# SaurabhIndi/unet-segmentation

Measured on AMD Instinct MI355X. Metric: training images/sec (512×512×1, batch=8) at 1/2/4/8 MI355X; IoU vs ref, higher is better.
Workload: dtype fp32; 1 GPU; U-Net train step 512x512x1, batch 8/GPU, fp32 GEMMs (fwd+WCE+bwd+SGD); global_batch=8, image=512, parallelism=dp1

## Files before the change

### include/unet_hip.h

```cpp
#ifndef UNET_HIP_H
#define UNET_HIP_H

#include <stddef.h>
#include <stdint.h>

#ifdef __cplusplus
extern "C" {
#endif

typedef void* unet_stream_t;

const char* unet_version(void);
const char* unet_last_error(void);

typedef struct unet_plan unet_plan;

unet_plan* unet_plan_create(int n, int c_in, int h, int w, int n_classes);

enum { UNET_PREC_FP32 = 0, UNET_PREC_BF16 = 1, UNET_PREC_BF16X3 = 2 };
unet_plan* unet_plan_create_ex(int n, int c_in, int h, int w, int n_classes, int precision);
int unet_plan_precision(const unet_plan* p);
void unet_plan_destroy(unet_plan* p);
int unet_plan_out_hw(const unet_plan* p, int* out_h, int* out_w);
size_t unet_plan_workspace_bytes(const unet_plan* p);
// ... 65 lines not shown
int unet_weight_map(const uint16_t* labels, int n, int h, int w, double w0, double sigma, float* weights,
                    double* weights64, void* ws, unet_stream_t stream);

size_t unet_weight_map_border_ws_bytes(int n, int h, int w);
int unet_weight_map_border(const uint16_t* labels, int n, int h, int w, double w0, double sigma, float* weights,
                           double* weights64, int32_t* d1sq, int32_t* d2sq, void* ws, unet_stream_t stream);

size_t unet_instance_masks_ws_bytes(int n, int h, int w);
int unet_instance_masks(const uint8_t* mask, int n, int h, int w, int min_size, uint16_t* labels, void* ws,
                        unet_stream_t stream);
size_t unet_rand_index_ws_bytes(int h, int w);
int unet_rand_index(const uint16_t* gt, const uint16_t* pred, int h, int w, double* out, void* ws,
                    unet_stream_t stream);

typedef struct unet_tracker unet_tracker;
unet_tracker* unet_tracker_create(int h, int w, double iou_track, double iou_division, int max_children);
void unet_tracker_destroy(unet_tracker* t);
size_t unet_tracker_ws_bytes(int h, int w);
int unet_tracker_add_frame(unet_tracker* t, const uint16_t* labels, int frame, void* ws, unet_stream_t stream);
int unet_tracker_step_host(unet_tracker* t, int frame, int n_curr, const int32_t* host_labels,
                           const int64_t* host_areas, const int64_t* host_inter);
int unet_tracker_num_tracks(const unet_tracker* t);
int unet_tracker_tracks(const unet_tracker* t, int32_t* host_out, int cap);
int unet_linear_sum_assignment(long long nr, long long nc, const double* host_cost, int64_t* host_row_ind,
                               int64_t* host_col_ind);

int unet_set_tuning(const char* key, int value);
size_t unet_tuning_report(char* buf, size_t len);
int unet_tuning_reset(void);
long long unet_slab_fallbacks(int reset);
long long unet_nondeterministic_sites(int reset);
long long unet_fused_bnb_sites(int reset);
long long unet_wgrad_oihw_sites(int reset);
int unet_tuning_save(const char* path);
int unet_tuning_load(const char* path);

int unet_conv3x3_fwd(const float* x, int n, int h, int w, int ci, const float* wt_oihw,
                     const float* bias, int co, const float* x_scale, const float* x_shift,
                     float* y, void* ws, unet_stream_t stream);
int unet_conv3x3_dgrad(const float* dy, int n, int h, int w, int ci, const float* wt_oihw,
                       int co, float* dx, void* ws, unet_stream_t stream);
int unet_conv3x3_wgrad(const float* x, const float* dy, int n, int h, int w, int ci, int co,
                       float* dw_oihw, float* db, void* ws, unet_stream_t stream);
size_t unet_conv_ws_bytes(int n, int h, int w, int ci, int co);
int unet_convT2_fwd(const float* x, int n, int h, int w, int ci, const float* wt, const float* bias,
                    int co, float* y, void* ws, unet_stream_t stream);
int unet_convT2_bwd(const float* x, const float* dy, int n, int h, int w, int ci, const float* wt,
                    int co, float* dx, float* dw, float* db, void* ws, unet_stream_t stream);
int unet_maxpool2_fwd(const float* x, int n, int h, int w, int c, float* y, uint8_t* arg,
                      unet_stream_t stream);
int unet_maxpool2_bwd(const float* dy, const uint8_t* arg, int n, int h, int w, int c, float* dx,
                      unet_stream_t stream);
int unet_bn_train_fwd(const float* x, int n, int h, int w, int c, const float* gamma,
                      const float* beta, float* running_mean, float* running_var, float* y,
                      float* save_mean, float* save_invstd, void* ws, unet_stream_t stream);
int unet_bn_train_bwd(const float* x, const float* dy, int n, int h, int w, int c,
                      const float* gamma, const float* save_mean, const float* save_invstd,
                      float* dx, float* dgamma, float* dbeta, void* ws, unet_stream_t stream);
size_t unet_bn_ws_bytes(int c);

size_t unet_bn_relu_ws_bytes(int n, int h, int w, int c);
int unet_bn_relu_fwd(const float* x, int n, int h, int w, int c, const float* gamma, const float* beta,
                     float* running_mean, float* running_var, int64_t* nbt, float momentum, float eps,
                     int training, int relu, float* y, float* save_mean, float* save_invstd, void* ws,
                     unet_stream_t stream);
int unet_bn_relu_bwd(const float* x, const float* y, const float* dy, int n, int h, int w, int c,
// ... 20 lines not shown
```

### unet-segmentation_amd/csrc/igemm.hip

```cpp
#include <algorithm>
#include <cstdio>
#include <cstdlib>

#include "gemm_common.h"
#include "ring_common.h"

namespace unet {
constexpr int igemm_minw(int BM, int BN, int WM, int WN, int BK) {
  const int lds = 2 * (BM + BN) * (BK + 4) * 4 + WM * 3 * BN * 4;
  int blocks = 163840 / lds;
  if (blocks > 8) blocks = 8;
  int w = blocks * WM * WN * 64 / 256;
  if (WM * WN >= 8 && w > 2) w = 2;
  return w < 1 ? 1 : (w > 8 ? 8 : w);
}

template <int BM, int BN, int WM, int WN, int BK, int ABL = 0, int PF = 1>
__global__ __launch_bounds__(WM * WN * 64, igemm_minw(BM, BN, WM, WN, BK)) void k_igemm(const IgemmArgs args) {
  constexpr int NT = WM * WN * 64;
  constexpr int LDK = BK + 4;
  constexpr int TM = BM / (WM * 32), TN = BN / (WN * 32);
  constexpr int C4 = BK / 4;
  constexpr int RPP = NT / C4;
  constexpr int AV = BM / RPP, BV = BN / RPP;
// ... 944 lines not shown
  return g_num_cus;
}

int ablation_env(const char* name) {
  const char* v = getenv(name);
  if (!v || !*v) return 0;
#ifdef UNET_ABLATIONS
  return atoi(v);
#else
  fprintf(stderr, "unet_hip: %s=%s ignored (timing ablations need a build with -DUNET_ABLATIONS: make ABLATIONS=1)\n",
          name, v);
  return 0;
#endif
}

static int env_int(const char* name, int dflt) {
  const char* v = getenv(name);
  return v ? atoi(v) : dflt;
}
int g_tune_igemm = env_int("UNET_IGEMM_VARIANT", -1);
int g_tune_wgrad = env_int("UNET_WGRAD_VARIANT", -1);
std::atomic<long long> g_slab_fallbacks{0};
int g_wino_max = env_int("UNET_WINO_MAX", 4);
int g_wino_dgrad_max = env_int("UNET_WINO_DGRAD_MAX", 4);
int g_wino_wgrad_max = env_int("UNET_WINO_WGRAD_MAX", 6);
int g_wino4_fwd_min_cg = env_int("UNET_WINO4_FWD_MIN_CG", 128);
int g_wino4_fwd_small_cg = env_int("UNET_WINO4_FWD_SMALL_CG", 0);
template <int BM, int BN, int WM, int WN, int BK>
static hipError_t go_igemm(const IgemmArgs& a, hipStream_t s) {
  if (a.N % BN != 0 || a.K % BK != 0 || a.a.Cg % BK != 0 || a.a.c_split % BK != 0) return hipErrorInvalidValue;
  if (a.batch > 1) {
    if (a.ksplit > 1 || a.batch_rows < 1) return hipErrorInvalidValue;
    dim3 grid((a.batch_rows + BM - 1) / BM, a.N / BN, a.batch);
    hipLaunchKernelGGL((k_igemm<BM, BN, WM, WN, BK>), grid, dim3(WM * WN * 64), 0, s, a);
    return hipGetLastError();
  }
  dim3 grid((a.M + BM - 1) / BM, a.N / BN, a.ksplit > 1 ? a.ksplit : 1);
  hipLaunchKernelGGL((k_igemm<BM, BN, WM, WN, BK>), grid, dim3(WM * WN * 64), 0, s, a);
  return hipGetLastError();
}

template <int BM, int BN, int WM, int WN>
static hipError_t go_igemm_g(const IgemmArgs& a, hipStream_t s) {
  if (a.N % BN != 0 || a.K % 16 != 0 || a.a.Cg % 16 != 0 || a.a.c_split % 16 != 0) return hipErrorInvalidValue;
  static bool attr = false;
  const size_t full = igemm_g_smem<BM, BN>(1024);
  if (!attr) {
    hipError_t e = hipFuncSetAttribute(reinterpret_cast<const void*>(&k_igemm_g<BM, BN, WM, WN>),
                                       hipFuncAttributeMaxDynamicSharedMemorySize, (int)full);
    if (e != hipSuccess) return e;
    attr = true;
  }
  const bool tf = a.a.s[0].scale != nullptr || (a.a.c_split < a.a.Cg && a.a.s[1].scale != nullptr);
  if (tf && a.a.Cg > 1024) return hipErrorInvalidValue;
  const size_t smem = igemm_g_smem<BM, BN>(tf ? a.a.Cg : 0);
  dim3 grid((a.M + BM - 1) / BM, a.N / BN, a.ksplit > 1 ? a.ksplit : 1);
  hipLaunchKernelGGL((k_igemm_g<BM, BN, WM, WN>), grid, dim3(WM * WN * 64), smem, s, a);
  return hipGetLastError();
}

template <int TH, int TW, int BN, int WM, int WN, int MINW>
static hipError_t go_halo32(const IgemmArgs& a, hipStream_t s) {
  if (a.b == nullptr || a.N % BN != 0 || a.a.Cg % 16 != 0 || a.a.c_split % 16 != 0 || a.a.taps_h != 3 ||
      a.a.taps_w != 3 || a.a.stride != 1 || a.K != 9 * a.a.Cg)
    return hipErrorInvalidValue;
  constexpr size_t smem = conv3_f32_smem<TH, TW, BN>();
// ... 351 lines not shown
```

### unet-segmentation_amd/csrc/ops.hip

```cpp
#include <algorithm>
#include <cerrno>
#include <string>

#include "../../include/unet_hip.h"
#include "unet_internal.h"

using namespace unet;

namespace unet {
extern int g_tune_igemm, g_tune_wgrad, g_autotune, g_force_split, g_force_tile, g_concurrent, g_wino_max,
    g_wino_dgrad_max, g_wino_wgrad_max, g_bf16_norm, g_bn_fold, g_wino4_fwd_min_cg, g_wino4_fwd_small_cg,
    g_maxpool_vec8, g_wgrad_fwd_u;
hipError_t launch_fill(float* p, size_t n, float v, hipStream_t s);
hipError_t launch_pair_sum(const double* st, int g, int c, float* out, hipStream_t s);
}

namespace {
thread_local std::string g_op_err;
inline size_t al256(size_t b) { return (b + 255) / 256 * 256; }
int g_op_prec = UNET_PREC_FP32;
int g_op_a16 = 0;

hipError_t op_b_to_bf16(IgemmArgs& a, size_t n, void* scratch, hipStream_t s) {
  if (g_op_prec == UNET_PREC_FP32) return hipSuccess;
// ... 4 lines not shown
  a.bl = bl;
  a.b = nullptr;
  return e;
}
}

namespace {
__global__ void k_relu_mask(const float* __restrict__ dy, const float* __restrict__ y, long long n4,
                            float* __restrict__ dz) {
  for (long long i = blockIdx.x * (long long)blockDim.x + threadIdx.x; i < n4; i += (long long)gridDim.x * blockDim.x) {
    const float4 g = reinterpret_cast<const float4*>(dy)[i], v = reinterpret_cast<const float4*>(y)[i];
    reinterpret_cast<float4*>(dz)[i] =
        make_float4(v.x > 0.f ? g.x : 0.f, v.y > 0.f ? g.y : 0.f, v.z > 0.f ? g.z : 0.f, v.w > 0.f ? g.w : 0.f);
  }
}

__global__ void k_bn_eval_stats(int C, const float* rm, const float* rv, float eps, float* mean, float* invstd) {
  const int c = blockIdx.x * blockDim.x + threadIdx.x;
  if (c >= C) return;
  mean[c] = rm[c];
  invstd[c] = (float)(1.0 / sqrt((double)rv[c] + (double)eps));
}
}

#define OPCK(x)                                                           \
  do {                                                                    \
    hipError_t e_ = (x);                                                  \
    if (e_ != hipSuccess) return e_ == hipErrorInvalidValue ? -EINVAL : -EIO; \
  } while (0)

extern "C" {

static size_t op_wino_bytes(int ci, int co) { return al256(sizeof(float) * 36 * (size_t)ci * co); }
static void op_set_wino(IgemmArgs& a, void* ws, size_t ws_bytes, int ci, int co) {
  a.wino_ws = reinterpret_cast<float*>(reinterpret_cast<char*>(ws) + ws_bytes - op_wino_bytes(ci, co));
  a.wino_ws_bytes = op_wino_bytes(ci, co);
}

static size_t op_wgrad_wino_bytes(int n, int h, int w, int ci, int co) {
  return al256(wino_ws_bytes_grid(n, h, w, ci, co));
}
static size_t op_wgrad_slab_bytes(int n, int h, int w, int ci, int co) {
  const long long t4 = (long long)n * ((h + 3) / 4) * ((w + 3) / 4);
  return al256(sizeof(float) * 64 * (size_t)std::min<long long>(64, (t4 + 255) / 256) * ci * co);
}
static size_t op_wgrad_extra_bytes(int n, int h, int w, int ci, int co) {
  const size_t b = op_wgrad_wino_bytes(n, h, w, ci, co) + op_wgrad_slab_bytes(n, h, w, ci, co);
  return b <= ((size_t)256 << 20) ? b : 0;
}

size_t unet_conv_ws_bytes(int n, int h, int w, int ci, int co) {
  const size_t wb = al256(sizeof(float) * 9 * (size_t)ci * co);
  const size_t pad = al256(sizeof(float) * (size_t)n * (h + 2) * (w + 2) * co);
  const size_t misc = al256(sizeof(float) * 4 * co) + al256(sizeof(double) * kStatGroups * 2 * co);
  const size_t x16 = al256(sizeof(uint16_t) * (size_t)n * h * w * ci);
  return 2 * wb + pad + misc + x16 + op_wgrad_extra_bytes(n, h, w, ci, co) + op_wino_bytes(ci, co);
}

int unet_conv3x3_fwd(const float* x, int n, int h, int w, int ci, const float* wt, const float* bias, int co,
                     const float* xs, const float* xb, float* y, void* ws, unet_stream_t st) {
  if (ci % 16 || co % 64 || h < 3 || w < 3) return -EINVAL;
  hipStream_t s = reinterpret_cast<hipStream_t>(st);
  float* wf = reinterpret_cast<float*>(ws);
  OPCK(launch_pack_conv(wt, co, ci, 3, 3, wf, nullptr, s));
  IgemmArgs a;
  Src x0;
  x0.ptr = x;
  x0.H = h;
  x0.W = w;
  x0.C = ci;
  x0.scale = xs;
  x0.shift = xb;
  if (g_op_prec == UNET_PREC_BF16 && g_op_a16) {
    const size_t wb = al256(sizeof(float) * 9 * (size_t)ci * co);
    const size_t off = 2 * wb + al256(sizeof(float) * (size_t)n * (h + 2) * (w + 2) * co) +
                       al256(sizeof(float) * 4 * co) + al256(sizeof(double) * kStatGroups * 2 * co);
    uint16_t* x16 = reinterpret_cast<uint16_t*>(reinterpret_cast<char*>(ws) + off);
    OPCK(launch_f2bf(x, x16, (size_t)n * h * w * ci, s));
    x0.ptr = reinterpret_cast<const float*>(x16);
    x0.h16 = 1;
  }
  a.a.s[0] = a.a.s[1] = x0;
  a.a.Cg = a.a.c_split = ci;
  a.a.taps_h = a.a.taps_w = 3;
  a.a.Hg = h - 2;
  a.a.Wg = w - 2;
  a.a.nimg = n;
  a.b = wf;
  a.M = n * (h - 2) * (w - 2);
  a.N = co;
  a.K = 9 * ci;
  a.e.bias = bias;
  a.e.d[0] = Dst{y, h - 2, w - 2, co, 0, 0};
  op_set_wino(a, ws, unet_conv_ws_bytes(n, h, w, ci, co), ci, co);
  OPCK(op_b_to_bf16(a, 9 * (size_t)ci * co, reinterpret_cast<char*>(ws) + al256(sizeof(float) * 9 * (size_t)ci * co),
                    s));
  OPCK(launch_igemm(a, s));
  return 0;
}

int unet_conv3x3_dgrad(const float* dy, int n, int h, int w, int ci, const float* wt, int co, float* dx, void* ws,
                       unet_stream_t st) {
  if (ci % 64 || co % 16 || h < 3 || w < 3) return -EINVAL;
  hipStream_t s = reinterpret_cast<hipStream_t>(st);
  char* p = reinterpret_cast<char*>(ws);
  const size_t wb = al256(sizeof(float) * 9 * (size_t)ci * co);
  float* wf = reinterpret_cast<float*>(p);
  float* wd = reinterpret_cast<float*>(p + wb);
  float* dyp = reinterpret_cast<float*>(p + 2 * wb);
  float* coef = reinterpret_cast<float*>(p + 2 * wb + al256(sizeof(float) * (size_t)n * (h + 2) * (w + 2) * co));
  OPCK(launch_pack_conv(wt, co, ci, 3, 3, wf, wd, s));
  OPCK(launch_fill(coef, co, 1.f, s));
  OPCK(launch_fill(coef + co, 3 * (size_t)co, 0.f, s));
  const int dy16 = g_op_prec == UNET_PREC_BF16 && g_op_a16;
  OPCK(launch_bnb_apply(dy, dy, coef, n, h - 2, w - 2, co, dyp, 2, s, dy16, 0));
  IgemmArgs a;
  Src d;
  d.ptr = dyp;
  d.h16 = dy16;
  d.H = h + 2;
  d.W = w + 2;
  d.C = co;
  a.a.s[0] = a.a.s[1] = d;
  a.a.Cg = a.a.c_split = co;
  a.a.taps_h = a.a.taps_w = 3;
  a.a.Hg = h;
  a.a.Wg = w;
  a.a.nimg = n;
  a.b = wd;
  a.M = n * h * w;
  a.N = ci;
  a.K = 9 * co;
  a.e.d[0] = Dst{dx, h, w, ci, 0, 0};
  op_set_wino(a, ws, unet_conv_ws_bytes(n, h, w, ci, co), ci, co);
  OPCK(op_b_to_bf16(a, 9 * (size_t)ci * co, wf, s));
  OPCK(launch_igemm(a, s));
  return 0;
}

int unet_conv3x3_wgrad(const float* x, const float* dy, int n, int h, int w, int ci, int co, float* dw, float* db,
                       void* ws, unet_stream_t st) {
  if (ci % 64 || co % 64 || h < 3 || w < 3) return -EINVAL;
  hipStream_t s = reinterpret_cast<hipStream_t>(st);
  char* p = reinterpret_cast<char*>(ws);
  const size_t wb = al256(sizeof(float) * 9 * (size_t)ci * co);
  float* dwp = reinterpret_cast<float*>(p);
  double* st2 = reinterpret_cast<double*>(p + 2 * wb + al256(sizeof(float) * (size_t)n * (h + 2) * (w + 2) * co) +
                                          al256(sizeof(float) * 4 * co));
  OPCK(hipMemsetAsync(dwp, 0, sizeof(float) * 9 * (size_t)ci * co, s));
  WgradArgs a;
  Src d;
  d.ptr = dy;
  d.H = h - 2;
  d.W = w - 2;
  d.C = co;
  a.ga.s[0] = a.ga.s[1] = d;
  a.ga.Cg = a.ga.c_split = co;
  a.ga.Hg = h - 2;
  a.ga.Wg = w - 2;
  a.ga.nimg = n;
  Src xs;
  xs.ptr = x;
  xs.H = h;
  xs.W = w;
  xs.C = ci;
  a.gb.s[0] = a.gb.s[1] = xs;
  a.gb.Cg = a.gb.c_split = ci;
// ... 320 lines not shown
                      unet_stream_t st) {
  OPCK(launch_sgd(p, g, buf, n, lr, mom, gscale, first, reinterpret_cast<hipStream_t>(st)));
  return 0;
}

int unet_iou_counts(const uint8_t* a, const uint8_t* b, size_t n, unsigned long long* out, unet_stream_t st) {
  OPCK(launch_iou(a, b, n, out, reinterpret_cast<hipStream_t>(st)));
  return 0;
}

int unet_set_tuning(const char* key, int value) {
  if (!key) return -EINVAL;
  const std::string k(key);
  if (k == "igemm_variant") g_tune_igemm = value;
  else if (k == "wgrad_variant") g_tune_wgrad = value;
  else if (k == "autotune") g_autotune = value;
  else if (k == "force_split") g_force_split = value;
  else if (k == "force_tile") g_force_tile = value;
  else if (k == "concurrent") g_concurrent = value;
  else if (k == "wino_max") g_wino_max = value;
  else if (k == "bf16_norm") g_bf16_norm = value;
  else if (k == "bn_fold") g_bn_fold = value != 0;
  else if (k == "wino_dgrad_max") g_wino_dgrad_max = value;
  else if (k == "wino_wgrad_max") g_wino_wgrad_max = value;
  else if (k == "wino4_fwd_min_cg") g_wino4_fwd_min_cg = value;
  else if (k == "wino4_fwd_small_cg") g_wino4_fwd_small_cg = value;
  else if (k == "op_a16") g_op_a16 = value != 0;
  else if (k == "maxpool_vec8") g_maxpool_vec8 = value;
  else if (k == "bnb_fuse") g_bnb_fuse = value;
  else if (k == "wgrad_early_u") g_wgrad_early_u = value;
  else if (k == "wgrad_fwd_u") g_wgrad_fwd_u = value;
  else if (k == "wgrad_plane") g_wgrad_plane = value;
  else if (k == "wgrad_oihw") g_wgrad_oihw = value;
  else if (k == "deterministic") g_deterministic = value != 0;
  else if (k == "op_precision") {
    if (value != UNET_PREC_FP32 && value != UNET_PREC_BF16 && value != UNET_PREC_BF16X3) return -EINVAL;
    g_op_prec = value;
  } else return -EINVAL;
  return 0;
}

int unet_tile_gather(const float* image, int c, int h, int w, int tile_in, int tile_out, int top, int left, int nx,
                     int first, int stride, int ntiles, float* tiles, unet_stream_t st) {
  if (!image || !tiles) return -EINVAL;
  OPCK(launch_tile_gather(image, c, h, w, tile_in, tile_out, top, left, nx, first, stride, ntiles, tiles,
                          reinterpret_cast<hipStream_t>(st)));
  return 0;
}

int unet_tile_scatter(const float* tile_logits, int k, int tile_out, int nx, int first, int stride, int ntiles, int h,
                      int w, float* logits, uint8_t* mask, unet_stream_t st) {
  if (!tile_logits) return -EINVAL;
  OPCK(launch_tile_scatter(tile_logits, k, tile_out, nx, first, stride, ntiles, h, w, logits, mask,
                           reinterpret_cast<hipStream_t>(st)));
  return 0;
}

size_t unet_instance_masks_ws_bytes(int n, int h, int w) {
  return n > 0 && h > 0 && w > 0 ? instance_masks_ws_bytes(n, h, w) : 0;
}

int unet_instance_masks(const uint8_t* mask, int n, int h, int w, int min_size, uint16_t* labels, void* ws,
                        unet_stream_t st) {
  if (!mask || !labels || !ws) return -EINVAL;
  OPCK(launch_instance_masks(mask, n, h, w, min_size, labels, ws, reinterpret_cast<hipStream_t>(st)));
  return 0;
// ... 66 lines not shown
```

### unet-segmentation_amd/csrc/plan.hip

```cpp
#include <cerrno>
#include <cstdio>
#include <cstdlib>
#include <cstring>
#include <algorithm>
#include <array>
#include <map>
#include <mutex>
#include <string>
#include <vector>

#include "../../include/unet_hip.h"
#include "unet_internal.h"

using namespace unet;

namespace unet {
extern int g_wino_max, g_wino_dgrad_max, g_wino_wgrad_max, g_wino4_fwd_min_cg, g_wino4_fwd_small_cg;
int g_autotune = getenv("UNET_AUTOTUNE") ? atoi(getenv("UNET_AUTOTUNE")) : 1;
int g_concurrent = getenv("UNET_CONCURRENT") ? atoi(getenv("UNET_CONCURRENT")) : 1;
int g_bf16_norm = getenv("UNET_BF16_NORM") ? atoi(getenv("UNET_BF16_NORM")) : 0;
int g_bn_fold = getenv("UNET_BN_FOLD") ? atoi(getenv("UNET_BN_FOLD")) : 1;
int g_force_split = 0;
int g_force_tile = 0;
int g_deterministic = getenv("UNET_DETERMINISTIC") ? atoi(getenv("UNET_DETERMINISTIC")) : 0;
// ... 1344 lines not shown
    return -EINVAL;
  }
  if (!p->side || !p->side_pending) return 0;
  CK(hipEventRecord(p->ev_join, p->side));
  CK(hipStreamWaitEvent(reinterpret_cast<hipStream_t>(stream), p->ev_join, 0));
  p->side_pending = false;
  return 0;
}

size_t unet_tuning_report(char* buf, size_t len) {
  std::string r;
  {
    std::lock_guard<std::mutex> lk(g_tune_mu);
    for (const auto& kv : g_tune_log) r += kv.second + "\n";
  }
  if (buf && len > 0) {
    const size_t k = std::min(len - 1, r.size());
    memcpy(buf, r.data(), k);
    buf[k] = 0;
  }
  return r.size() + 1;
}

long long unet_nondeterministic_sites(int reset) {
  return reset ? g_nondet_sites.exchange(0) : g_nondet_sites.load();
}

long long unet_fused_bnb_sites(int reset) {
  return reset ? unet::g_fused_bnb_sites.exchange(0) : unet::g_fused_bnb_sites.load();
}
long long unet_wgrad_oihw_sites(int reset) {
  return reset ? unet::g_wgrad_oihw_sites.exchange(0) : unet::g_wgrad_oihw_sites.load();
}
long long unet_slab_fallbacks(int reset) {
  return reset ? g_slab_fallbacks.exchange(0) : g_slab_fallbacks.load();
}

int unet_tuning_reset(void) {
  std::lock_guard<std::mutex> lk(g_tune_mu);
  g_tuned.clear();
  g_tune_log.clear();
  return 0;
}

int unet_tuning_save(const char* path) {
  if (!path) return -EINVAL;
  std::lock_guard<std::mutex> lk(g_tune_mu);
  FILE* f = fopen(path, "w");
  if (!f) return -errno;
  for (const auto& kv : g_tuned) fprintf(f, "%s\t%d\t%d\n", kv.first.c_str(), kv.second.tile, kv.second.split);
  fclose(f);
  return (int)g_tuned.size();
}

int unet_tuning_load(const char* path) {
  if (!path) return -EINVAL;
  std::lock_guard<std::mutex> lk(g_tune_mu);
  return tune_db_read(path, true);
}

int unet_plan_set_timing(unet_plan* p, int enable) {
  if (!p) return -EINVAL;
  p->timing = enable != 0;
  return 0;
}

// ... 65 lines not shown
```

### unet-segmentation_amd/csrc/unet_internal.h

```cpp
#pragma once
#include <hip/hip_runtime.h>
#include <cstddef>
#include <cstdint>
#include <atomic>
#include <string>
#include <vector>

namespace unet {

constexpr int kMaxInChannels = 4096;
constexpr int kMaxClassCount = 4096;

struct Src {
  const float* ptr = nullptr;
  int H = 0, W = 0, C = 0;
  int oy = 0, ox = 0;
  const float* scale = nullptr;
  const float* shift = nullptr;
  int h16 = 0;
};

struct Gather {
  Src s[2];
  int c_split = 0;
// ... 24 lines not shown
  const float* bn_shift = nullptr;
  const float* bn_mean = nullptr;
  const float* bn_invstd = nullptr;
  double* bstats = nullptr;
  double* colsum1 = nullptr;
};

constexpr int kStatGroups = 64;

struct IgemmArgs {
  Gather a;
  const float* b = nullptr;
  const uint16_t* bh = nullptr;
  const uint16_t* bl = nullptr;
  int M, N, K;
  Epilogue e;
  int ksplit = 1;
  float* slab = nullptr;
  float* wino_ws = nullptr;
  size_t wino_ws_bytes = 0;
  int batch = 1;
  int batch_rows = 0;
  long long batch_b = 0;
  struct { int tile = -1, split = 1; } wino_choice;
  int fwd = 0;
};

extern std::atomic<long long> g_slab_fallbacks;
extern int g_deterministic;
extern int g_bnb_fuse;
extern int g_wgrad_early_u;
extern int g_wgrad_plane;
extern int g_wgrad_oihw;
extern std::atomic<long long> g_nondet_sites;

struct WgradArgs {
  Gather ga;
  Gather gb;
  int Mo, No;
  int P;
  int pix_per_split;
  float* out;
  float* out_oihw = nullptr;
  float* slab = nullptr;
  size_t slab_bytes = 0;
  int accumulate = 0;
  int bf16 = 0;
  int split = 0;
  int batch = 1;
  long long batch_a = 0, batch_b = 0, batch_out = 0;
  float* wino_ws = nullptr;
  size_t wino_ws_bytes = 0;
  const float* vd_pre = nullptr;
  int u_ready = 0;
  int abl = 0;
};

struct GemmChoice {
  int tile = -1;
  int split = 1;
};

enum class IgemmFamily {
  Reg,
  Halo,
  Conv3Dma,
// ... 96 lines not shown
size_t bnb_wino6_vd_bytes(int n, int h, int w, int c);
hipError_t launch_bnb_wino6_dy(const float* dz, const float* y, const float* coef, int n, int h, int w, int c,
                               float* dypad, float* vd, hipStream_t s);
bool conv3_ring_fits(const IgemmArgs& a, const IgemmTile& t);
bool gemm_ring_fits(const IgemmArgs& a, const IgemmTile& t);
size_t conv3_flat_sk_slab_bytes(const IgemmArgs& a);
int num_cus();

int ablation_env(const char* name);
hipError_t launch_igemm(const IgemmArgs& a, hipStream_t s);
hipError_t launch_igemm_v(const IgemmArgs& a, hipStream_t s, GemmChoice c);
int igemm_heuristic_tile(const IgemmArgs& a);
bool igemm_tile_fits(const IgemmArgs& a, int tile);
long long igemm_tile_count(const IgemmArgs& a, int tile);
int igemm_tile_slots(int tile);
size_t igemm_slab_bytes(const IgemmArgs& a, int ksplit);
std::string igemm_key(const IgemmArgs& a);
std::string wgrad_key(const WgradArgs& a);
std::vector<GemmChoice> igemm_candidates(const IgemmArgs& a, size_t slab_bytes);
std::vector<GemmChoice> wgrad_candidates(const WgradArgs& a);
bool wgrad_choice_deterministic(const GemmChoice& g);
hipError_t launch_wgrad(const WgradArgs& a, hipStream_t s);
hipError_t launch_wgrad_v(const WgradArgs& a, hipStream_t s, GemmChoice c);
bool wgrad_tile_fits(const WgradArgs& a, int tile);
bool reg_tile_fits(const IgemmArgs& a, const IgemmTile& t);
bool halo_tile_fits(const IgemmArgs& a, const IgemmTile& t);
bool wgrad3_fits(const WgradArgs& a);
hipError_t launch_slab_reduce(const float* slab, int splits, int batch, size_t plane, long long batch_out, float* out,
                              hipStream_t s);
int wgrad_splits(const WgradArgs& a, const WgradTile& t, int per_cu, int& pps);
bool wgrad_slab_fits(const WgradArgs& a, int splits);
bool wgrad_plane_applies(const WgradArgs& a, int bm, int bn);
hipError_t launch_wgrad_plane(const WgradArgs& a, hipStream_t s, dim3 grid, int bm, int bn);
hipError_t launch_f2bf(const float* in, uint16_t* out, size_t n, hipStream_t s, uint16_t* lo = nullptr);

hipError_t launch_tile_gather(const float* img, int c, int h, int w, int ti, int to, int top, int left, int nx,
                              int first, int stride, int ntiles, float* tiles, hipStream_t s);
hipError_t launch_tile_scatter(const float* lt, int k, int to, int nx, int first, int stride, int ntiles, int h,
                               int w, float* full, uint8_t* mask, hipStream_t s);

size_t instance_masks_ws_bytes(int n, int h, int w);
hipError_t launch_instance_masks(const uint8_t* mask, int n, int h, int w, int min_size, uint16_t* out, void* ws,
                                 hipStream_t s);
size_t rand_index_ws_bytes(int h, int w);
hipError_t launch_rand_index(const uint16_t* g, const uint16_t* p, int h, int w, double* out, void* ws,
                             hipStream_t s);

void set_last_error(const std::string& s);

size_t weight_map_ws_bytes(int n);
hipError_t launch_weight_map(const uint16_t* lab, int n, int h, int w, double w0, double sigma, float* out,
                             double* out64, void* ws, hipStream_t s);
size_t weight_map_border_ws_bytes(int n, int h, int w);
hipError_t launch_weight_map_border(const uint16_t* lab, int n, int h, int w, double w0, double sigma, float* out,
                                    double* out64, int32_t* d1sq, int32_t* d2sq, void* ws, hipStream_t s);

size_t elastic_ws_bytes(int n, int h, int w);
hipError_t launch_elastic(const uint8_t* img, const uint16_t* lab, int n, int h, int w, const double* noise,
                          double alpha, double sigma, float* x_out, uint8_t* t_out, uint8_t* img_out, uint16_t* ids_out,
                          void* ws, hipStream_t s);

hipError_t launch_conv_first_fwd(const float* x_nchw, int n, int ci, int h, int w,
                                 const float* wt_oihw, const float* bias, int co, float* y,
                                 double* stats, hipStream_t s, int out_h16 = 0, int relu = 0);
hipError_t launch_fold_bn(const float* w, long long K, int rows, const float* scale, const float* shift,
                          const float* bias, float* wout, float* bias_out, hipStream_t s);
// ... 78 lines not shown
```

### unet-segmentation_amd/csrc/winograd.hip

```cpp
#include <algorithm>
#include <cstdlib>

#include "gemm_common.h"
#include "ring_common.h"

namespace unet {

__global__ void k_wino_w(const float* __restrict__ b, int N, int Cg, float* __restrict__ v) {
  const long long i = blockIdx.x * (long long)blockDim.x + threadIdx.x;
  if (i >= (long long)N * Cg) return;
  const int n = (int)(i / Cg), c = (int)(i - (long long)n * Cg);
  float g[3][3];
#pragma unroll
  for (int t = 0; t < 9; ++t) g[t / 3][t % 3] = b[((size_t)n * 9 + t) * Cg + c];
  float tg[4][3];
#pragma unroll
  for (int k = 0; k < 3; ++k) {
    tg[0][k] = g[0][k];
    tg[1][k] = 0.5f * (g[0][k] + g[1][k] + g[2][k]);
    tg[2][k] = 0.5f * (g[0][k] - g[1][k] + g[2][k]);
    tg[3][k] = g[2][k];
  }
  const size_t plane = (size_t)N * Cg, o = (size_t)n * Cg + c;
#pragma unroll
// ... 606 lines not shown
    }
  }
}

static size_t wino_bytes(int P, long long T, int Cg, int N) {
  auto al = [](size_t b) { return (b + 255) / 256 * 256; };
  return al((size_t)P * T * Cg * 4) + al((size_t)P * T * N * 4) + al((size_t)P * N * Cg * 4);
}
size_t wino_ws_bytes(long long T, int Cg, int N) { return wino_bytes(16, T, Cg, N); }
size_t wino_ws_bytes_grid(int nimg, int H, int W, int Cg, int N) {
  const long long t2 = (long long)nimg * ((H + 1) / 2) * ((W + 1) / 2);
  const long long t4 = (long long)nimg * ((H + 3) / 4) * ((W + 3) / 4);
  const long long t6 = (long long)nimg * ((H + 5) / 6) * ((W + 5) / 6);
  const size_t a = wino_bytes(16, t2, Cg, N), b = wino_bytes(36, t4, Cg, N), c = wino_bytes(64, t6, Cg, N);
  return std::max(a, std::max(b, c));
}

bool wino_applies(const IgemmArgs& a, int mt) {
  const Gather& g = a.a;
  if (a.b == nullptr || a.bh != nullptr || g.taps_h != 3 || g.taps_w != 3 || g.stride != 1 || a.K != 9 * g.Cg ||
      g.Cg % 4 || g.c_split % 4 || a.N % 64 || g.s[0].h16 || g.s[1].h16 || a.e.shuffle_co)
    return false;
  for (int k = 0; k < 2; ++k) {
    const Dst& d = a.e.d[k];
    if (k == 1 && a.e.n_split >= a.N) break;
    if (d.h16 || d.oy || d.ox || d.H != g.Hg || d.W != g.Wg || d.C % 4) return false;
  }
  if (a.e.yref_h16 || a.e.n_split % 4) return false;
  const long long T = (long long)g.nimg * ((g.Hg + mt - 1) / mt) * ((g.Wg + mt - 1) / mt);
  if ((long long)(mt + 2) * (mt + 2) * T * std::max(g.Cg, a.N) * 4 >= (1ll << 32)) return false;
  return a.wino_ws != nullptr && wino_bytes((mt + 2) * (mt + 2), T, g.Cg, a.N) <= a.wino_ws_bytes;
}

hipError_t launch_wino(const IgemmArgs& a, hipStream_t s, int mt) {
  if (!wino_applies(a, mt)) return hipErrorInvalidValue;
  const Gather& g = a.a;
  const int P = (mt + 2) * (mt + 2);
  const int Th = (g.Hg + mt - 1) / mt, Tw = (g.Wg + mt - 1) / mt;
  const long long T = (long long)g.nimg * Th * Tw;
  char* w = reinterpret_cast<char*>(a.wino_ws);
  auto al = [](size_t b) { return (b + 255) / 256 * 256; };
  float* U = reinterpret_cast<float*>(w);
  float* Mm = reinterpret_cast<float*>(w + al((size_t)P * T * g.Cg * 4));
  float* V = reinterpret_cast<float*>(w + al((size_t)P * T * g.Cg * 4) + al((size_t)P * T * a.N * 4));
  const long long nw = (long long)a.N * g.Cg;
  if (mt == 2) {
    hipLaunchKernelGGL(k_wino_w, dim3((unsigned)((nw + 255) / 256)), dim3(256), 0, s, a.b, a.N, g.Cg, V);
    const long long ni = T * (g.Cg / 4);
    hipLaunchKernelGGL(k_wino_in, dim3((unsigned)((ni + 255) / 256)), dim3(256), 0, s, g, Th, Tw, T, U);
  } else if (mt == 4) {
    hipLaunchKernelGGL(k_wino4_w, dim3((unsigned)((nw + 255) / 256)), dim3(256), 0, s, a.b, a.N, g.Cg, V);
    launch_wino4_in(g, Th, Tw, T, U, s);
  } else {
    hipLaunchKernelGGL(k_wino6_w, dim3((unsigned)((nw + 255) / 256)), dim3(256), 0, s, a.b, a.N, g.Cg, V);
    launch_wino6_in(g, Th, Tw, T, U, s);
  }
  hipError_t e = hipGetLastError();
  if (e != hipSuccess) return e;
  {
    IgemmArgs q;
    Src u;
    u.ptr = U;
    u.H = 1;
    u.W = (int)(P * T);
    u.C = g.Cg;
    q.a.s[0] = q.a.s[1] = u;
    q.a.Cg = q.a.c_split = g.Cg;
    q.a.taps_h = q.a.taps_w = 1;
    q.a.Hg = 1;
    q.a.Wg = (int)(P * T);
    q.a.nimg = 1;
    q.b = V;
    q.M = (int)(P * T);
    q.N = a.N;
    q.K = g.Cg;
    q.e.d[0] = Dst{Mm, 1, (int)(P * T), a.N, 0, 0};
    q.batch = P;
    q.batch_rows = (int)T;
    q.batch_b = (long long)a.N * g.Cg;
    int tile = a.wino_choice.tile;
    if (tile <= 0 || !igemm_tile_fits(q, tile)) {
      const long long t256 = ((T + 255) / 256) * (a.N / 128) * P;
      tile = (a.N % 128 == 0 && t256 >= 2 * num_cus()) ? 4 : (a.N % 128 == 0 ? 1 : 8);
    }
    if ((e = launch_igemm_v(q, s, GemmChoice{tile, 1})) != hipSuccess) return e;
  }
  if (mt == 2) {
    const int C4 = a.N / 4, cgs = C4 < 64 ? C4 : 64, lanes = 256 / cgs;
    long long gx = (T + lanes * 4 - 1) / (lanes * 4);
    if (gx > 65535) gx = 65535;
    dim3 grid((unsigned)gx, (unsigned)((C4 + cgs - 1) / cgs));
    hipLaunchKernelGGL(k_wino_out, grid, dim3(256), 0, s, Mm, T, Th, Tw, a.N, g, a.e);
  } else {
    long long gx = (T + 15) / 16;
    if (gx > 65535) gx = 65535;
    dim3 grid((unsigned)gx, (unsigned)((a.N + 63) / 64));
    if (mt == 4) hipLaunchKernelGGL(k_wino4_out, grid, dim3(256), 0, s, Mm, T, Th, Tw, a.N, g, a.e);
    else hipLaunchKernelGGL(k_wino6_out, grid, dim3(256), 0, s, Mm, T, Th, Tw, a.N, g, a.e);
  }
  return hipGetLastError();
}

template <int CK>
__global__ void k_wino4f_w(const float* __restrict__ b, int N, int Cg, float* __restrict__ v) {
  const long long i = blockIdx.x * (long long)blockDim.x + threadIdx.x;
  if (i >= (long long)N * Cg) return;
  const int n = (int)(i / Cg), c = (int)(i - (long long)n * Cg);
  float tg[6][3];
#pragma unroll
  for (int k = 0; k < 3; ++k) {
    float col[3] = {b[((size_t)n * 9 + 0 + k) * Cg + c], b[((size_t)n * 9 + 3 + k) * Cg + c],
                    b[((size_t)n * 9 + 6 + k) * Cg + c]};
    float r[6];
// ... 1546 lines not shown
```

### unet-segmentation_amd/unet_amd/_lib.py

```python
from __future__ import annotations

import ctypes
import os

_HERE = os.path.dirname(os.path.abspath(__file__))
LIB_PATH = os.environ.get("UNET_HIP_LIB", os.path.join(_HERE, "libunet_hip.so"))

_vp = ctypes.c_void_p
_i = ctypes.c_int
_f = ctypes.c_float
_sz = ctypes.c_size_t

SIGNATURES = {
    "unet_version": (ctypes.c_char_p, []),
    "unet_last_error": (ctypes.c_char_p, []),
    "unet_plan_create": (_vp, [_i, _i, _i, _i, _i]),
    "unet_plan_create_ex": (_vp, [_i, _i, _i, _i, _i, _i]),
    "unet_plan_precision": (_i, [_vp]),
    "unet_plan_destroy": (None, [_vp]),
    "unet_plan_out_hw": (_i, [_vp, ctypes.POINTER(_i), ctypes.POINTER(_i)]),
    "unet_plan_workspace_bytes": (_sz, [_vp]),
    "unet_plan_forward_workspace_bytes": (_sz, [_vp]),
    "unet_plan_num_params": (_i, [_vp]),
    "unet_plan_num_grads": (_i, [_vp]),
# ... 38 lines not shown
    "unet_convT2_fwd": (_i, [_vp, _i, _i, _i, _i, _vp, _vp, _i, _vp, _vp, _vp]),
    "unet_convT2_bwd": (_i, [_vp, _vp, _i, _i, _i, _i, _vp, _i, _vp, _vp, _vp, _vp, _vp]),
    "unet_maxpool2_fwd": (_i, [_vp, _i, _i, _i, _i, _vp, _vp, _vp]),
    "unet_maxpool2_bwd": (_i, [_vp, _vp, _i, _i, _i, _i, _vp, _vp]),
    "unet_bn_train_fwd": (_i, [_vp, _i, _i, _i, _i, _vp, _vp, _vp, _vp, _vp, _vp, _vp, _vp, _vp]),
    "unet_bn_train_bwd": (_i, [_vp, _vp, _i, _i, _i, _i, _vp, _vp, _vp, _vp, _vp, _vp, _vp, _vp]),
    "unet_bn_ws_bytes": (_sz, [_i]),
    "unet_bn_relu_ws_bytes": (_sz, [_i, _i, _i, _i]),
    "unet_bn_relu_fwd": (_i, [_vp, _i, _i, _i, _i, _vp, _vp, _vp, _vp, _vp, _f, _f, _i, _i, _vp, _vp, _vp, _vp,
                              _vp]),
    "unet_bn_relu_bwd": (_i, [_vp, _vp, _vp, _i, _i, _i, _i, _vp, _vp, _vp, _i, _i, _vp, _vp, _vp, _vp, _vp]),
    "unet_conv_first_ws_bytes": (_sz, [_i, _i, _i, _i]),
    "unet_conv_first_fwd": (_i, [_vp, _i, _i, _i, _i, _vp, _vp, _vp, _vp]),
    "unet_conv_first_bwd": (_i, [_vp, _vp, _i, _i, _i, _i, _vp, _vp, _vp, _vp, _vp, _vp]),
    "unet_conv1x1_ws_bytes": (_sz, [_i]),
    "unet_conv1x1_fwd": (_i, [_vp, _i, _i, _i, _i, _vp, _vp, _i, _vp, _vp]),
    "unet_conv1x1_bwd": (_i, [_vp, _vp, _i, _i, _i, _i, _vp, _i, _vp, _vp, _vp, _vp, _vp]),
    "unet_peak_probe": (_i, [_i, _i, ctypes.POINTER(ctypes.c_double), _vp]),
    "unet_tracker_create": (_vp, [_i, _i, ctypes.c_double, ctypes.c_double, _i]),
    "unet_tracker_destroy": (None, [_vp]),
    "unet_tracker_ws_bytes": (_sz, [_i, _i]),
    "unet_tracker_add_frame": (_i, [_vp, _vp, _i, _vp, _vp]),
    "unet_tracker_step_host": (_i, [_vp, _i, _i, _vp, _vp, _vp]),
    "unet_tracker_num_tracks": (_i, [_vp]),
    "unet_tracker_tracks": (_i, [_vp, _vp, _i]),
    "unet_linear_sum_assignment": (_i, [ctypes.c_longlong, ctypes.c_longlong, _vp, _vp, _vp]),
    "unet_set_tuning": (_i, [ctypes.c_char_p, _i]),
    "unet_tuning_report": (_sz, [ctypes.c_char_p, _sz]),
    "unet_tuning_reset": (_i, []),
    "unet_slab_fallbacks": (ctypes.c_longlong, [_i]),
    "unet_nondeterministic_sites": (ctypes.c_longlong, [_i]),
    "unet_fused_bnb_sites": (ctypes.c_longlong, [_i]),
    "unet_wgrad_oihw_sites": (ctypes.c_longlong, [_i]),
    "unet_tuning_save": (_i, [ctypes.c_char_p]),
    "unet_tuning_load": (_i, [ctypes.c_char_p]),
}

_lib = None
_load_error = None


def load():
    global _lib, _load_error
    if _lib is not None:
        return _lib
    if _load_error is not None:
        raise RuntimeError(_load_error)
    try:
        lib = ctypes.CDLL(LIB_PATH, mode=ctypes.RTLD_GLOBAL)
    except OSError as e:
        _load_error = (f"libunet_hip.so could not be loaded from {LIB_PATH} ({e}); "
                       "build it with `python -c 'import __graft_entry__ as g; g.build()'`")
        raise RuntimeError(_load_error) from e
    for name, (res, args) in SIGNATURES.items():
        fn = getattr(lib, name)
        fn.restype = res
        fn.argtypes = args
    _lib = lib
    return lib


def last_error() -> str:
    msg = load().unet_last_error()
    return msg.decode() if msg else ""


def check(rc: int, what: str) -> None:
    if rc != 0:
        raise RuntimeError(f"{what} failed (rc={rc}): {last_error()}")


def ptr(t) -> int:
    return None if t is None else t.data_ptr()


def ptr_array(tensors):
    arr = (ctypes.c_void_p * len(tensors))()
    for i, t in enumerate(tensors):
        arr[i] = t.data_ptr()
    return arr


def stream_of(device=None):
    import torch
    return ctypes.c_void_p(torch.cuda.current_stream(device).cuda_stream)


_HASHED = ["igemm.hip", "igemm_bf16.hip", "conv3_dma.hip", "conv3_ring.hip", "winograd.hip", "elementwise.hip", "elastic.hip",
           "tiling.hip", "weightmap.hip", "postproc.hip", "track.hip", "ops.hip", "plan.hip", "wgrad3_ring.hip",
           "conv3_ring_pt.hip", "peak.hip", "gemm_ring.hip", "wgradT_ring.hip", "conv3_flat.hip", "conv3_c64.hip", "gemm_ring_p1.hip",
           "gemm_ring_p2.hip", "wgrad_plane.hip", "unet_internal.h", "gemm_common.h", "ring_common.h", "conv3_ring_kernel.h",
           os.path.join("..", "..", "include", "unet_hip.h")]


def source_hash() -> str:
    import hashlib
    h = hashlib.sha256()
    csrc = os.path.join(_HERE, "..", "csrc")
    for f in _HASHED:
        with open(os.path.join(csrc, f), "rb") as fh:
            h.update(fh.read())
    return h.hexdigest()[:16]


def build_identity() -> dict:
    v = load().unet_version().decode()
    built = v.rsplit(" src ", 1)[-1].split()[0] if " src " in v else "unknown"
    tree = source_hash()
    return {"version": v, "lib_src": built, "tree_src": tree, "src_match": built == tree,
            "ablation_build": v.endswith(" ablations")}


def slab_fallbacks(reset: bool = False) -> int:
    return int(load().unet_slab_fallbacks(1 if reset else 0))


def tuning_report() -> str:
    lib = load()
    n = lib.unet_tuning_report(None, 0)
    buf = ctypes.create_string_buffer(n)
    lib.unet_tuning_report(buf, n)
    return buf.value.decode()
```

Baseline: 312.1 images/s.

## Add DMA ring-buffered plane GEMM kernel for batched pointwise igemm launches

Adds a new k_igemm_plane kernel that takes batched 1x1/pointwise igemm cases (such as Winograd point-wise GEMMs) and streams A/B tiles into a multi-slot LDS ring with direct-to-LDS loads and vmcnt-based waits instead of the generic gather loader. It is on by default through an env/tuning flag and is used only when strict layout and alignment conditions hold. The change also adds a Winograd point-tile override knob and reworks Winograd workspace selection for forced wino tiles. The deeper pipeline costs LDS and occupancy, and the narrow applicability checks limit which calls take the new path.

Measured after the change: 317.7 images/s, median of 6. 1.8% higher.

```diff
diff --git a/include/unet_hip.h b/include/unet_hip.h
--- a/include/unet_hip.h
+++ b/include/unet_hip.h
@@ -121,6 +121,7 @@
 long long unet_nondeterministic_sites(int reset);
 long long unet_fused_bnb_sites(int reset);
 long long unet_wgrad_oihw_sites(int reset);
+long long unet_igemm_plane_launches(int reset);
 int unet_tuning_save(const char* path);
 int unet_tuning_load(const char* path);
 
diff --git a/unet-segmentation_amd/csrc/igemm.hip b/unet-segmentation_amd/csrc/igemm.hip
--- a/unet-segmentation_amd/csrc/igemm.hip
+++ b/unet-segmentation_amd/csrc/igemm.hip
@@ -1000,6 +1000,7 @@
   if (a.batch > 1) {
     if (a.ksplit > 1 || a.batch_rows < 1) return hipErrorInvalidValue;
     dim3 grid((a.batch_rows + BM - 1) / BM, a.N / BN, a.batch);
+    if (WM == 2 && WN == 2 && igemm_plane_applies(a, BM, BN, BK)) return launch_igemm_plane(a, s, grid, BM, BN, BK);
     hipLaunchKernelGGL((k_igemm<BM, BN, WM, WN, BK>), grid, dim3(WM * WN * 64), 0, s, a);
     return hipGetLastError();
   }
diff --git a/unet-segmentation_amd/csrc/igemm_plane.hip b/unet-segmentation_amd/csrc/igemm_plane.hip
--- /dev/null
+++ b/unet-segmentation_amd/csrc/igemm_plane.hip
@@ -0,0 +1,166 @@
+#include <atomic>
+#include <cstdlib>
+
+#include "gemm_common.h"
+#include "ring_common.h"
+
+namespace unet {
+
+namespace {
+constexpr int plane_minw(int BM, int BN, int BK) {
+  return BK == 32 ? 2 : (BM == 128 && BN == 128 ? 3 : 4);
+}
+constexpr int plane_ns(int BM, int BN, int BK) { return 163840 / plane_minw(BM, BN, BK) / ((BM + BN) * 64); }
+}
+
+template <int BM, int BN, int BK>
+__global__ __launch_bounds__(256, plane_minw(BM, BN, BK)) void k_igemm_plane(const IgemmArgs args) {
+  constexpr int WM = 2, WN = 2, NW = WM * WN, NT = NW * 64;
+  constexpr int TM = BM / (WM * 32), TN = BN / (WN * 32);
+  constexpr int G = BK / 16;
+  constexpr int NS = plane_ns(BM, BN, BK);
+  constexpr int ASZ = BM * 64, SUB = (BM + BN) * 64;
+  constexpr int PA = BM / (16 * NW), PB = BN / (16 * NW), D = PA + PB;
+  constexpr int AHEAD = NS - 2 * G;
+  constexpr int KH = BK / 2, KF = KH / 4;
+  static_assert(TM >= 1 && TN >= 1 && PA >= 1 && PB >= 1 && (G == 1 || G == 2), "tile");
+  static_assert(AHEAD >= 1 && D * AHEAD < 64 && NS * SUB <= 81920 && NS * SUB >= WM * 3 * BN * 4, "ring depth / vmcnt / LDS");
+  __shared__ __attribute__((aligned(1024))) unsigned char lds[NS * SUB];
+  const unsigned lds0 = (unsigned)(size_t)(lds_u8_t*)lds;
+
+  const int tid = threadIdx.x, lane = tid & 63;
+  const int wave = __builtin_amdgcn_readfirstlane(tid >> 6);
+  const int wm = wave / WN, wn = wave % WN;
+  int bx, by, bz;
+  xcd_block(bx, by, bz);
+  const int m0 = bz * args.batch_rows + bx * BM, n0 = by * BN;
+  const int M = (bz + 1) * args.batch_rows, K = args.K;
+  const int S = K / 16, nk = K / BK;
+
+  const unsigned rowb = (unsigned)K * 4u;
+  const int mlast = M - 1 - m0;
+  unsigned long long abase = uniform_u64(args.a.s[0].ptr + (size_t)m0 * K);
+  unsigned long long bbase = uniform_u64(args.b + (size_t)bz * args.batch_b + (size_t)n0 * K);
+  unsigned aoff[PA], boff[PB];
+#pragma unroll
+  for (int u = 0; u < PA; ++u) {
+    const int r = (wave * PA + u) * 16 + (lane >> 2);
+    aoff[u] = (unsigned)min(r, mlast) * rowb + (unsigned)(((lane & 3) ^ ((r >> 2) & 3)) * 16);
+  }
+#pragma unroll
+  for (int u = 0; u < PB; ++u) {
+    const int r = (wave * PB + u) * 16 + (lane >> 2);
+    boff[u] = (unsigned)r * rowb + (unsigned)(((lane & 3) ^ ((r >> 2) & 3)) * 16);
+  }
+  int issued = 0, islot = 0;
+  auto issue = [&] {
+    const unsigned dst = lds0 + (unsigned)islot * SUB;
+#pragma unroll
+    for (int u = 0; u < PA; ++u) dma_sv(aoff[u], abase, dst + (wave * PA + u) * 1024);
+#pragma unroll
+    for (int u = 0; u < PB; ++u) dma_sv(boff[u], bbase, dst + ASZ + (wave * PB + u) * 1024);
+    abase += 64;
+    bbase += 64;
+    ++issued;
+    islot = islot + 1 == NS ? 0 : islot + 1;
+  };
+
+  floatx16 acc[TM][TN];
+#pragma unroll
+  for (int i = 0; i < TM; ++i)
+#pragma unroll
+    for (int j = 0; j < TN; ++j)
+#pragma unroll
+      for (int r = 0; r < 16; ++r) acc[i][j][r] = 0.f;
+
+  const int h = lane >> 5, li = lane & 31;
+  const int sw = (li >> 2) & 3;
+  int cslot = 0;
+  auto compute = [&] {
+    int sub = cslot, c0 = 2 * h;
+    if constexpr (G == 2) {
+      const int nxt = cslot + 1 == NS ? 0 : cslot + 1;
+      sub = h ? nxt : cslot;
+      c0 = 0;
+    }
+    const float* As = reinterpret_cast<const float*>(lds + sub * SUB);
+    const float* Bs = reinterpret_cast<const float*>(lds + sub * SUB + ASZ);
+    float4 fa[TM][KF], fb[TN][KF];
+#pragma unroll
+    for (int i = 0; i < TM; ++i) {
+      const float* pr = As + (wm * TM * 32 + i * 32 + li) * 16;
+#pragma unroll
+      for (int f = 0; f < KF; ++f) fa[i][f] = ld4(pr + (((c0 + f) ^ sw) << 2));
+    }
+#pragma unroll
+    for (int j = 0; j < TN; ++j) {
+      const float* pr = Bs + (wn * TN * 32 + j * 32 + li) * 16;
+#pragma unroll
+      for (int f = 0; f < KF; ++f) fb[j][f] = ld4(pr + (((c0 + f) ^ sw) << 2));
+    }
+#pragma unroll
+    for (int s = 0; s < KH; ++s)
+#pragma unroll
+      for (int i = 0; i < TM; ++i)
+#pragma unroll
+        for (int j = 0; j < TN; ++j)
+          acc[i][j] = __builtin_amdgcn_mfma_f32_32x32x2f32(getc(fa[i][s >> 2], s & 3), getc(fb[j][s >> 2], s & 3),
+                                                           acc[i][j], 0, 0, 0);
+    cslot += G;
+    if (cslot >= NS) cslot -= NS;
+  };
+
+#pragma unroll
+  for (int t = 0; t < NS - G; ++t)
+    if (t < S) issue();
+  for (int kc = 0; kc < nk; ++kc) {
+    if (S - (kc + 1) * G >= AHEAD) vm_wait<D * AHEAD>();
+    else vm_wait<0>();
+    raw_barrier();
+#pragma unroll
+    for (int t = 0; t < G; ++t)
+      if (issued < S) issue();
+    compute();
+  }
+  __syncthreads();
+  igemm_finish<BM, BN, WM, WN, NT>(args, acc, m0, n0, wm, wn, tid, reinterpret_cast<float*>(lds), LinearRows{m0, M},
+                                   nullptr, bz);
+}
+
+int g_igemm_plane = getenv("UNET_IGEMM_PLANE") ? atoi(getenv("UNET_IGEMM_PLANE")) : 1;
+std::atomic<long long> g_igemm_plane_launches{0};
+
+static bool plane_tile(int bm, int bn, int bk) {
+  return (bk == 16 && ((bm == 128 && bn == 128) || (bm == 64 && bn == 128) || (bm == 128 && bn == 64))) ||
+         (bk == 32 && bn == 128 && (bm == 128 || bm == 64));
+}
+
+bool igemm_plane_applies(const IgemmArgs& a, int bm, int bn, int bk) {
+  if (!g_igemm_plane || !plane_tile(bm, bn, bk) || a.batch <= 1 || a.ksplit != 1 || a.batch_rows < 1) return false;
+  const Gather& g = a.a;
+  const Src& s = g.s[0];
+  if (g.taps_h != 1 || g.taps_w != 1 || g.stride != 1 || g.Hg != 1 || g.nimg != 1) return false;
+  if (g.c_split != g.Cg || s.C != g.Cg || a.K != g.Cg || a.K % bk != 0 || a.N % bn != 0) return false;
+  if (s.scale || s.h16 || a.bh || !a.b || !s.ptr) return false;
+  const long long rows = (long long)a.batch * a.batch_rows;
+  if (s.H != 1 || s.oy != 0 || s.ox != 0 || s.W != g.Wg || rows != g.Wg || rows != a.M) return false;
+  const Epilogue& e = a.e;
+  const Dst& d = e.d[0];
+  if (e.shuffle_co || e.n_split < a.N || d.h16 || d.oy != 0 || d.ox != 0 || d.H != 1 || d.W != g.Wg) return false;
+  if (((reinterpret_cast<size_t>(s.ptr) | reinterpret_cast<size_t>(a.b)) & 15) != 0 || (a.batch_b * 4) % 16 != 0)
+    return false;
+  return (long long)(bm > bn ? bm : bn) * a.K * 4 < (1ll << 32);
+}
+
+hipError_t launch_igemm_plane(const IgemmArgs& a, hipStream_t s, dim3 grid, int bm, int bn, int bk) {
+  if (bm == 128 && bn == 128 && bk == 16) hipLaunchKernelGGL((k_igemm_plane<128, 128, 16>), grid, dim3(256), 0, s, a);
+  else if (bm == 64 && bn == 128 && bk == 16) hipLaunchKernelGGL((k_igemm_plane<64, 128, 16>), grid, dim3(256), 0, s, a);
+  else if (bm == 128 && bn == 64 && bk == 16) hipLaunchKernelGGL((k_igemm_plane<128, 64, 16>), grid, dim3(256), 0, s, a);
+  else if (bm == 128 && bn == 128 && bk == 32) hipLaunchKernelGGL((k_igemm_plane<128, 128, 32>), grid, dim3(256), 0, s, a);
+  else if (bm == 64 && bn == 128 && bk == 32) hipLaunchKernelGGL((k_igemm_plane<64, 128, 32>), grid, dim3(256), 0, s, a);
+  else return hipErrorInvalidValue;
+  ++g_igemm_plane_launches;
+  return hipGetLastError();
+}
+
+}
diff --git a/unet-segmentation_amd/csrc/ops.hip b/unet-segmentation_amd/csrc/ops.hip
--- a/unet-segmentation_amd/csrc/ops.hip
+++ b/unet-segmentation_amd/csrc/ops.hip
@@ -60,7 +60,17 @@
 extern "C" {
 
 static size_t op_wino_bytes(int ci, int co) { return al256(sizeof(float) * 36 * (size_t)ci * co); }
-static void op_set_wino(IgemmArgs& a, void* ws, size_t ws_bytes, int ci, int co) {
+static size_t op_wgrad_wino_bytes(int n, int h, int w, int ci, int co);
+static size_t op_wgrad_extra_bytes(int n, int h, int w, int ci, int co);
+static void op_set_wino(IgemmArgs& a, void* ws, int n, int h, int w, int ci, int co) {
+  const size_t ws_bytes = unet_conv_ws_bytes(n, h, w, ci, co);
+  const IgemmTile* forced = igemm_tile(g_tune_igemm);
+  if (forced && forced->family == IgemmFamily::Wino && op_wgrad_extra_bytes(n, h, w, ci, co)) {
+    a.wino_ws = reinterpret_cast<float*>(reinterpret_cast<char*>(ws) + ws_bytes - op_wino_bytes(ci, co) -
+                                         op_wgrad_extra_bytes(n, h, w, ci, co));
+    a.wino_ws_bytes = op_wgrad_wino_bytes(n, h, w, ci, co);
+    return;
+  }
   a.wino_ws = reinterpret_cast<float*>(reinterpret_cast<char*>(ws) + ws_bytes - op_wino_bytes(ci, co));
   a.wino_ws_bytes = op_wino_bytes(ci, co);
 }
@@ -120,7 +130,7 @@
   a.K = 9 * ci;
   a.e.bias = bias;
   a.e.d[0] = Dst{y, h - 2, w - 2, co, 0, 0};
-  op_set_wino(a, ws, unet_conv_ws_bytes(n, h, w, ci, co), ci, co);
+  op_set_wino(a, ws, n, h, w, ci, co);
   OPCK(op_b_to_bf16(a, 9 * (size_t)ci * co, reinterpret_cast<char*>(ws) + al256(sizeof(float) * 9 * (size_t)ci * co),
                     s));
   OPCK(launch_igemm(a, s));
@@ -160,7 +170,7 @@
   a.N = ci;
   a.K = 9 * co;
   a.e.d[0] = Dst{dx, h, w, ci, 0, 0};
-  op_set_wino(a, ws, unet_conv_ws_bytes(n, h, w, ci, co), ci, co);
+  op_set_wino(a, ws, n, h, w, ci, co);
   OPCK(op_b_to_bf16(a, 9 * (size_t)ci * co, wf, s));
   OPCK(launch_igemm(a, s));
   return 0;
@@ -547,6 +557,8 @@
   else if (k == "wgrad_fwd_u") g_wgrad_fwd_u = value;
   else if (k == "wgrad_plane") g_wgrad_plane = value;
   else if (k == "wgrad_oihw") g_wgrad_oihw = value;
+  else if (k == "igemm_plane") g_igemm_plane = value;
+  else if (k == "wino_point_tile") g_wino_point_tile = value;
   else if (k == "deterministic") g_deterministic = value != 0;
   else if (k == "op_precision") {
     if (value != UNET_PREC_FP32 && value != UNET_PREC_BF16 && value != UNET_PREC_BF16X3) return -EINVAL;
diff --git a/unet-segmentation_amd/csrc/plan.hip b/unet-segmentation_amd/csrc/plan.hip
--- a/unet-segmentation_amd/csrc/plan.hip
+++ b/unet-segmentation_amd/csrc/plan.hip
@@ -1400,6 +1400,9 @@
 long long unet_wgrad_oihw_sites(int reset) {
   return reset ? unet::g_wgrad_oihw_sites.exchange(0) : unet::g_wgrad_oihw_sites.load();
 }
+long long unet_igemm_plane_launches(int reset) {
+  return reset ? unet::g_igemm_plane_launches.exchange(0) : unet::g_igemm_plane_launches.load();
+}
 long long unet_slab_fallbacks(int reset) {
   return reset ? g_slab_fallbacks.exchange(0) : g_slab_fallbacks.load();
 }
diff --git a/unet-segmentation_amd/csrc/unet_internal.h b/unet-segmentation_amd/csrc/unet_internal.h
--- a/unet-segmentation_amd/csrc/unet_internal.h
+++ b/unet-segmentation_amd/csrc/unet_internal.h
@@ -80,6 +80,9 @@
 extern int g_wgrad_early_u;
 extern int g_wgrad_plane;
 extern int g_wgrad_oihw;
+extern int g_igemm_plane;
+extern std::atomic<long long> g_igemm_plane_launches;
+extern int g_wino_point_tile;
 extern std::atomic<long long> g_nondet_sites;
 
 struct WgradArgs {
@@ -242,6 +245,8 @@
 bool wgrad_slab_fits(const WgradArgs& a, int splits);
 bool wgrad_plane_applies(const WgradArgs& a, int bm, int bn);
 hipError_t launch_wgrad_plane(const WgradArgs& a, hipStream_t s, dim3 grid, int bm, int bn);
+bool igemm_plane_applies(const IgemmArgs& a, int bm, int bn, int bk);
+hipError_t launch_igemm_plane(const IgemmArgs& a, hipStream_t s, dim3 grid, int bm, int bn, int bk);
 hipError_t launch_f2bf(const float* in, uint16_t* out, size_t n, hipStream_t s, uint16_t* lo = nullptr);
 
 hipError_t launch_tile_gather(const float* img, int c, int h, int w, int ti, int to, int top, int left, int nx,
diff --git a/unet-segmentation_amd/csrc/winograd.hip b/unet-segmentation_amd/csrc/winograd.hip
--- a/unet-segmentation_amd/csrc/winograd.hip
+++ b/unet-segmentation_amd/csrc/winograd.hip
@@ -662,6 +662,13 @@
   return a.wino_ws != nullptr && wino_bytes((mt + 2) * (mt + 2), T, g.Cg, a.N) <= a.wino_ws_bytes;
 }
 
+int g_wino_point_tile = -1;
+static bool wino_point_tile_ok(int id) {
+  for (int t : {1, 2, 3, 4, 6, 7, 8, 9})
+    if (t == id) return true;
+  return false;
+}
+
 hipError_t launch_wino(const IgemmArgs& a, hipStream_t s, int mt) {
   if (!wino_applies(a, mt)) return hipErrorInvalidValue;
   const Gather& g = a.a;
@@ -709,6 +716,7 @@
     q.batch_rows = (int)T;
     q.batch_b = (long long)a.N * g.Cg;
     int tile = a.wino_choice.tile;
+    if (wino_point_tile_ok(g_wino_point_tile) && igemm_tile_fits(q, g_wino_point_tile)) tile = g_wino_point_tile;
     if (tile <= 0 || !igemm_tile_fits(q, tile)) {
       const long long t256 = ((T + 255) / 256) * (a.N / 128) * P;
       tile = (a.N % 128 == 0 && t256 >= 2 * num_cus()) ? 4 : (a.N % 128 == 0 ? 1 : 8);
diff --git a/unet-segmentation_amd/unet_amd/_lib.py b/unet-segmentation_amd/unet_amd/_lib.py
--- a/unet-segmentation_amd/unet_amd/_lib.py
+++ b/unet-segmentation_amd/unet_amd/_lib.py
@@ -94,6 +94,7 @@
     "unet_nondeterministic_sites": (ctypes.c_longlong, [_i]),
     "unet_fused_bnb_sites": (ctypes.c_longlong, [_i]),
     "unet_wgrad_oihw_sites": (ctypes.c_longlong, [_i]),
+    "unet_igemm_plane_launches": (ctypes.c_longlong, [_i]),
     "unet_tuning_save": (_i, [ctypes.c_char_p]),
     "unet_tuning_load": (_i, [ctypes.c_char_p]),
 }
@@ -151,7 +152,7 @@
 _HASHED = ["igemm.hip", "igemm_bf16.hip", "conv3_dma.hip", "conv3_ring.hip", "winograd.hip", "elementwise.hip", "elastic.hip",
            "tiling.hip", "weightmap.hip", "postproc.hip", "track.hip", "ops.hip", "plan.hip", "wgrad3_ring.hip",
            "conv3_ring_pt.hip", "peak.hip", "gemm_ring.hip", "wgradT_ring.hip", "conv3_flat.hip", "conv3_c64.hip", "gemm_ring_p1.hip",
-           "gemm_ring_p2.hip", "wgrad_plane.hip", "unet_internal.h", "gemm_common.h", "ring_common.h", "conv3_ring_kernel.h",
+           "gemm_ring_p2.hip", "wgrad_plane.hip", "igemm_plane.hip", "unet_internal.h", "gemm_common.h", "ring_common.h", "conv3_ring_kernel.h",
            os.path.join("..", "..", "include", "unet_hip.h")]
 
 
```
